# SamsungLabs/nb-asr

Measured on NVIDIA B200. Metric: train_utterances_per_sec, higher is better.
Workload: dtype bf16

## Files before the change

include/nbasr.h:

```cpp
#ifndef NBASR_H
#define NBASR_H

#include <stdint.h>

#ifdef __cplusplus
extern "C" {
#endif

#define NBASR_F32 0
#define NBASR_BF16 1
#define NBASR_F16 2
#define NBASR_PAD_L 8
#define NBASR_PAD_R 4
#define NBASR_MAX_ADD 3

typedef struct nbasr_epilogue {
  const float* bias;
  int32_t relu20;
  float drop_p;
  uint64_t drop_seed;
  const uint64_t* drop_step;
  int32_t n_add;
  const void* add[NBASR_MAX_ADD];
  int32_t add_dtype;
// ... 47 lines not shown
  const void* x;
  int32_t B, T, Tp, C, cpg, ktaps, off0, dstep;
  const void* w;
  int32_t w_packed;
  nbasr_epilogue epi;
} nbasr_gconv;

int nbasr_gconv_fwd(const nbasr_gconv* p, void* stream);
int nbasr_gconv_chain(const nbasr_gconv* nodes, int n, int fused, void* work, int64_t work_bytes, void* stream);
int64_t nbasr_gconv_chain_work_bytes(int B, int T, int C, int cpg, int n);
int nbasr_pack_gconv_dgrad(const float* w, float* wt, int C, int cpg, int ktaps, void* stream);
int nbasr_pack_gconv_mma(const float* w, void* out, int out_dtype, int C, int cpg, int ktaps, int transposed, void* stream);
int64_t nbasr_gconv_mma_pack_elems(int C, int cpg, int ktaps);
int nbasr_gconv_wgrad(int dtype, const void* dz, const void* x, int B, int T, int Tp, int C, int cpg,
                      int ktaps, int off0, int dstep, float* dw, float* dbias, void* stream);

int nbasr_eltwise(int src_dtype, const void* src, int64_t ld_src, int B, int T, int Tp, int C,
                  const nbasr_epilogue* epi, void* stream);

int nbasr_colsum(int dtype, const void* x, int B, int T, int Tp, int C, float* out, void* stream);

int nbasr_layernorm_fwd(int dtype, const void* x, void* y, int B, int T, int Tp, int C,
                        const float* gamma, const float* beta, float eps, float* mean, float* rstd,
                        float out_scale, void* y2, void* stream);
int nbasr_layernorm_bwd(int dtype, const void* dy, const void* x, int x_dtype, float x_scale, const float* mean,
                        const float* rstd, const float* gamma, int B, int T, int Tp, int C, void* dx, void* dx2,
                        const uint32_t* mask2, float scale2, int64_t mask_rows, int mask2_w, float* dgamma,
                        float* dbeta, void* stream);

int nbasr_transpose_in(const float* audio, void* out, int dtype, int B, int F, int T, int Tp, float scale, void* stream);
// ... 86 lines not shown
```

nb_asr_b200/_lib.py:

```python
import ctypes as C
import os

from . import _build

F32, BF16, F16 = 0, 1, 2
PAD_L, PAD_R = 8, 4
MAX_ADD = 3

_vp, _i32, _i64, _f32, _u64 = C.c_void_p, C.c_int32, C.c_int64, C.c_float, C.c_uint64


class Epilogue(C.Structure):
    _fields_ = [('bias', _vp), ('relu20', _i32), ('drop_p', _f32), ('drop_seed', _u64), ('drop_step', _vp),
                ('n_add', _i32), ('add', _vp * MAX_ADD), ('add_dtype', _i32), ('out', _vp), ('out_dtype', _i32),
                ('ld_out', _i64), ('mask_out', _vp), ('out2', _vp), ('out2_dtype', _i32), ('mask2', _vp),
                ('scale2', _f32), ('mask_rows', _i64), ('mask_w', _i32), ('mask2_w', _i32), ('accumulate', _i32),
                ('acc_scale', _f32), ('bias_scale', _f32), ('relu_hi', _f32)]


class Gemm(C.Structure):
    _fields_ = [('dtype', _i32), ('a', _vp), ('a_bs', _i64), ('a_rs', _i64), ('nb', _i32), ('nr', _i32),
                ('K', _i32), ('N', _i32), ('w', _vp), ('ldw', _i64), ('o_r0', _i64), ('o_bs', _i64),
                ('o_rs', _i64), ('epi', Epilogue)]

# ... 15 lines not shown
class GateLayer(C.Structure):
    _fields_ = [('mask', _vp), ('mask_rows', _i64), ('w', _i32), ('C', _i32), ('Tp', _i32), ('T', _i32), ('s', _i32),
                ('reserved', _i32)]


_SIGS = {
    'nbasr_gemm_tn': [C.POINTER(Gemm), _vp],
    'nbasr_gemm_wgrad': [C.POINTER(Wgrad), _vp],
    'nbasr_gconv_fwd': [C.POINTER(GConv), _vp],
    'nbasr_gconv_chain': [C.POINTER(GConv), C.c_int, C.c_int, _vp, _i64, _vp],
    'nbasr_gconv_chain_work_bytes': [C.c_int] * 5,
    'nbasr_pack_gconv_dgrad': [_vp, _vp, C.c_int, C.c_int, C.c_int, _vp],
    'nbasr_pack_gconv_mma': [_vp, _vp, C.c_int, C.c_int, C.c_int, C.c_int, C.c_int, _vp],
    'nbasr_gconv_mma_pack_elems': [C.c_int, C.c_int, C.c_int],
    'nbasr_gconv_wgrad': [C.c_int, _vp, _vp] + [C.c_int] * 8 + [_vp, _vp, _vp],
    'nbasr_eltwise': [C.c_int, _vp, _i64, C.c_int, C.c_int, C.c_int, C.c_int, C.POINTER(Epilogue), _vp],
    'nbasr_colsum': [C.c_int, _vp, C.c_int, C.c_int, C.c_int, C.c_int, _vp, _vp],
    'nbasr_layernorm_fwd': [C.c_int, _vp, _vp, C.c_int, C.c_int, C.c_int, C.c_int, _vp, _vp, _f32, _vp, _vp, _f32, _vp, _vp],
    'nbasr_layernorm_bwd': [C.c_int, _vp, _vp, C.c_int, _f32, _vp, _vp, _vp, C.c_int, C.c_int, C.c_int, C.c_int, _vp, _vp, _vp,
                            _f32, _i64, C.c_int, _vp, _vp, _vp],
    'nbasr_transpose_in': [_vp, _vp, C.c_int, C.c_int, C.c_int, C.c_int, C.c_int, _f32, _vp],
    'nbasr_transpose_out': [_vp, _vp, C.c_int, C.c_int, C.c_int, C.c_int, _vp],
    'nbasr_param_stats': [_vp, _vp, _vp, _vp, C.c_int, _i64, _vp, _vp, _vp],
    'nbasr_row_gram': [_vp, C.c_int, _i64, _i64, _vp, _vp, _vp, _vp],
    'nbasr_gate_gram': [_vp, C.c_int, _vp, C.c_int, _vp, _vp, _vp],
    'nbasr_gate_gram_work_elems': [C.c_int],
    'nbasr_pack_weight': [_vp, _vp, C.c_int, C.c_int, C.c_int, C.c_int, C.c_int, C.c_int, _i64, _i64, _i64, _vp],
    'nbasr_convert': [_vp, _vp, C.c_int, _i64, _vp],
    'nbasr_lstm_fwd': [_vp, _vp, C.c_int, C.c_int, C.c_int, _vp, C.c_int, _i64, _i64, _i64, _vp, _vp, _vp, _vp, _vp],
    'nbasr_lstm_bwd': [_vp, _i64, _i64, _i64, _vp, _vp, _vp, C.c_int, C.c_int, C.c_int, _vp, _vp, _vp, _vp, _vp],
# ... 60 lines not shown
```

nb_asr_b200/csrc/gconv.cu:

```cuda
#include <algorithm>

#include "common.cuh"
#include "kernels.h"

namespace {

constexpr int G_TT = 64;
constexpr int G_FB = 16;
constexpr int G_MAXHALO = 12;
constexpr int G_NT = 256;

__host__ __device__ inline int slab_channels(int cpg) {
  return cpg == 10 ? 160 : 96;
}
__host__ __device__ inline int wpitch(int cpg, int ktaps) {
  int p = cpg * ktaps;
  return (p & 1) ? p : p + 1;
}

template <typename T>
__global__ void __launch_bounds__(G_NT) gconv_fwd_kernel(nbasr_gconv p) {
  extern __shared__ float smem[];
  const int CS = slab_channels(p.cpg);
  const int halo = (p.ktaps - 1) * p.dstep;
// ... 69 lines not shown
  for (int item = tid; item < G_TT * nch; item += G_NT) {
    int r = item / nch, ch = item % nch;
    int t = t0 + r;
    if (t >= p.T) continue;
    float v[32];
#pragma unroll
    for (int i = 0; i < 32; ++i) v[i] = (ch * 32 + i < cs) ? os[r * (CS + 1) + ch * 32 + i] : 0.f;
    int64_t rho = (int64_t)b * p.Tp + NBASR_PAD_L + t;
    epilogue_chunk(p.epi, rho, c_lo + ch * 32, p.C, v);
  }
}

constexpr int W_PAIRS = 7;
constexpr int W_FB = 8;

template <typename T>
__global__ void __launch_bounds__(G_NT) gconv_wgrad_kernel(const T* __restrict__ dz, const T* __restrict__ x, int B,
                                                           int Tt, int Tp, int C, int cpg, int ktaps, int off0,
                                                           int dstep, float* __restrict__ dw) {
  extern __shared__ float smem[];
  const int CS = slab_channels(cpg);
  const int halo = (ktaps - 1) * dstep;
  float* xs = smem;
  float* ds = xs + (G_TT + G_MAXHALO) * CS;
  const int tid = threadIdx.x;
  const int c_lo = blockIdx.x * CS;
  const int cs = min(CS, C - c_lo);
  const int b = blockIdx.y;
  const int npairs = cs * cpg;
  float acc[W_PAIRS][7];
#pragma unroll
  for (int q = 0; q < W_PAIRS; ++q)
#pragma unroll
    for (int j = 0; j < 7; ++j) acc[q][j] = 0.f;
  const int vec = cs >> 3;
  for (int t0 = 0; t0 < Tt; t0 += G_TT) {
    __syncthreads();
    for (int idx = tid; idx < (G_TT + halo) * vec; idx += G_NT) {
      int r = idx / vec, g8 = idx % vec;
      int t = t0 + off0 + r;
      float v[8];
      if (t >= 0 && t < Tt) load8(x + ((int64_t)b * Tp + NBASR_PAD_L + t) * C + c_lo + g8 * 8, v);
      else {
#pragma unroll
        for (int i = 0; i < 8; ++i) v[i] = 0.f;
      }
#pragma unroll
      for (int i = 0; i < 8; ++i) xs[r * CS + g8 * 8 + i] = v[i];
    }
    for (int idx = tid; idx < G_TT * vec; idx += G_NT) {
      int r = idx / vec, g8 = idx % vec;
      int t = t0 + r;
      float v[8];
      if (t < Tt) load8(dz + ((int64_t)b * Tp + NBASR_PAD_L + t) * C + c_lo + g8 * 8, v);
      else {
#pragma unroll
        for (int i = 0; i < 8; ++i) v[i] = 0.f;
      }
#pragma unroll
      for (int i = 0; i < 8; ++i) ds[r * CS + g8 * 8 + i] = v[i];
    }
    __syncthreads();
#pragma unroll
// ... 90 lines not shown
  if (packed) return sm100_gconv_chain(nodes, n, fused, work, work_bytes, as_stream(stream));
  for (int i = 0; i < n; ++i)
    if (nbasr_gconv_fwd(nodes + i, stream)) return 1;
  return 0;
}

int64_t nbasr_gconv_chain_work_bytes(int B, int T, int C, int cpg, int n) { return sm100_gconv_chain_work_bytes(B, T, C, cpg, n); }

int nbasr_pack_gconv_dgrad(const float* w, float* wt, int C, int cpg, int ktaps, void* stream) {
  int total = C * cpg * ktaps;
  pack_gconv_dgrad_kernel<<<(total + 255) / 256, 256, 0, as_stream(stream)>>>(w, wt, C, cpg, ktaps);
  NBASR_CHECK_LAUNCH();
  return 0;
}

int nbasr_gconv_wgrad(int dtype, const void* dz, const void* x, int B, int T, int Tp, int C, int cpg, int ktaps,
                      int off0, int dstep, float* dw, float* dbias, void* stream) {
  NBASR_REQUIRE(cpg == 6 || cpg == 8 || cpg == 10 || cpg == 12, "cpg");
  NBASR_REQUIRE(ktaps <= 7 && (dstep == 1 || dstep == 2), "taps");
  if (B <= 0 || T <= 0) return 0;
  if (dtype == NBASR_BF16 && !nbasr_env_flag(NBASR_ENV_FORCE_SIMT))
    return sm100_gconv_wgrad(dz, x, B, T, Tp, C, cpg, ktaps, off0, dstep, dw, dbias, as_stream(stream));
  if (dbias && nbasr_colsum(dtype, dz, B, T, Tp, C, dbias, stream)) return 1;
  int CS = slab_channels(cpg);
  dim3 grid((C + CS - 1) / CS, B);
  size_t sm = wgrad_smem(cpg);
  if (dtype == NBASR_BF16) {
    static DevOnce attr;
    if (!attr) { cudaFuncSetAttribute(gconv_wgrad_kernel<bf16>, cudaFuncAttributeMaxDynamicSharedMemorySize, 200 * 1024); attr = true; }
    gconv_wgrad_kernel<bf16><<<grid, G_NT, sm, as_stream(stream)>>>((const bf16*)dz, (const bf16*)x, B, T, Tp, C, cpg, ktaps, off0, dstep, dw);
  } else {
    static DevOnce attr;
    if (!attr) { cudaFuncSetAttribute(gconv_wgrad_kernel<float>, cudaFuncAttributeMaxDynamicSharedMemorySize, 200 * 1024); attr = true; }
    gconv_wgrad_kernel<float><<<grid, G_NT, sm, as_stream(stream)>>>((const float*)dz, (const float*)x, B, T, Tp, C, cpg, ktaps, off0, dstep, dw);
  }
  NBASR_CHECK_LAUNCH();
  return 0;
}

}
```

nb_asr_b200/csrc/gconv_sm100.cu:

```cuda
#include <cuda.h>

#include "common.cuh"
#include "kernels.h"
#include "sm100_ptx.cuh"
#include "gconv_sm100.cuh"

using namespace sm100;

namespace {

struct GcFwdArgs {
  int B, T, C, OUT, ktaps, dstep, off0;
  int nslabs, ntiles, tiles_per_utt, nlanes, nstage, no_prefetch, w_stable, f16;
  nbasr_epilogue epi;
  int64_t Tp;
};


__global__ void __launch_bounds__(FWD_THREADS, 2)
gconv_mma_fwd_kernel(const __grid_constant__ CUtensorMap tmX, const __grid_constant__ CUtensorMap tmW,
                     const __grid_constant__ CUtensorMap tmO, const __grid_constant__ CUtensorMap tmO2, const GcFwdArgs p) {
  extern __shared__ uint8_t smem_raw[];
  const uint32_t base = (smem_u32(smem_raw) + 1023u) & ~1023u;
  uint8_t* al = smem_raw + (base - smem_u32(smem_raw));
// ... 212 lines not shown
  __syncthreads();
  if (warp == W_MMA) {
    tcgen05_fence_after();
    tmem_dealloc(tm, 256);
  }
}

constexpr int DZROWS = 136;
constexpr int DZ_BYTES = DZROWS * 128;
constexpr int WG_STAGE = DZ_BYTES + A_BYTES;
constexpr int WG_SMEM = NSTAGE * WG_STAGE + 1024 + 256;

struct GcWgArgs {
  int B, T, C, cpg, OUT, ktaps, dstep, off0;
  int nslabs, nchunks, nunits, nlanes, dbg;
  float* dw;
  float* dbias;
};

__global__ void __launch_bounds__(GC_THREADS, 2)
gconv_mma_wgrad_kernel(const __grid_constant__ CUtensorMap tmDZ, const __grid_constant__ CUtensorMap tmX, const GcWgArgs p) {
  extern __shared__ uint8_t smem_raw[];
  const uint32_t base = (smem_u32(smem_raw) + 1023u) & ~1023u;
  uint8_t* al = smem_raw + (base - smem_u32(smem_raw));
  const uint32_t bar0 = base + NSTAGE * WG_STAGE;
  auto full_bar = [&](int s) { return bar0 + 8u * s; };
  auto empty_bar = [&](int s) { return bar0 + 8u * (NSTAGE + s); };
  const uint32_t tfull = bar0 + 8u * (2 * NSTAGE);
  auto ready_bar = [&](int s) { return bar0 + 8u * (2 * NSTAGE + 1 + s); };
  uint32_t* tptr = reinterpret_cast<uint32_t*>(al + NSTAGE * WG_STAGE + 8 * (3 * NSTAGE + 2));
  const int warp = uniform_warp_idx(), lane = threadIdx.x & 31;
  const int slab = blockIdx.x % p.nslabs;
  const int lane_id = blockIdx.x / p.nslabs;
  const int c0 = slab * p.OUT;
  const int cbox = c0 & ~7, coff = c0 - cbox;
  const int npairs = (p.ktaps + 1) / 2;

  if (warp == 4 && lane == 0) {
    prefetch_tmap(&tmDZ);
    prefetch_tmap(&tmX);
    for (int s = 0; s < NSTAGE; ++s) { mbar_init(full_bar(s), 1); mbar_init(empty_bar(s), 1); mbar_init(ready_bar(s), 1); }
    mbar_init(tfull, 1);
    fence_barrier_init();
  }
  if (warp == 5) tmem_alloc(smem_u32(tptr), 256);
  pdl_launch_dependents();
  tcgen05_fence_before();
  __syncthreads();
  tcgen05_fence_after();
  const uint32_t tm = *tptr;
  pdl_wait();
  const bool has_work = lane_id < p.nunits;

  if (warp == 4) {
    if (lane == 0) {
      int stage = 0;
// ... 3 lines not shown
        mbar_wait(empty_bar(stage), phase ^ 1);
        mbar_expect_tx(full_bar(stage), DZ_BYTES + A_BYTES);
        const uint32_t sa = base + stage * WG_STAGE;
        tma_load_3d(sa, &tmDZ, full_bar(stage), cbox, NBASR_PAD_L + t0 - p.dstep, b);
        tma_load_3d(sa + DZ_BYTES, &tmX, full_bar(stage), cbox, NBASR_PAD_L + t0 + p.off0, b);
        if (++stage == NSTAGE) { stage = 0; phase ^= 1; }
      }
    }
  } else if (warp == 5) {
    if (has_work) {
      const uint32_t idesc = make_idesc(128, 64 * npairs, 1, 1);
      int stage = 0;
      uint32_t phase = 0;
      bool first = true;
      for (int u = lane_id; u < p.nunits; u += p.nlanes) {
        mbar_wait(p.dbias ? ready_bar(stage) : full_bar(stage), phase);
        const uint32_t sa = base + stage * WG_STAGE;
        tcgen05_fence_after();
        const uint64_t ad0 = make_smem_desc(sa, (uint32_t)p.dstep * 128u, 1024);
        const uint64_t bd0 = make_smem_desc(sa + DZ_BYTES, 2u * (uint32_t)p.dstep * 128u, 1024);
        if (elect_one()) {
#pragma unroll
          for (int k = 0; k < GT / 16; ++k)
            if (!(p.dbg & 2048) || k == 0) umma_bf16(tm, ad0 + (uint64_t)(k * 128), bd0 + (uint64_t)(k * 128), idesc, (!first || k > 0) ? 1u : 0u);
          umma_commit(empty_bar(stage));
        }
        __syncwarp();
        first = false;
        if (++stage == NSTAGE) { stage = 0; phase ^= 1; }
      }
      if (elect_one()) umma_commit(tfull);
      __syncwarp();
    }
  } else if (has_work) {
    if (warp == 0 && p.dbias) {
      int stage = 0;
      uint32_t phase = 0;
      for (int u = lane_id; u < p.nunits; u += p.nlanes) {
        mbar_wait(full_bar(stage), phase);
        uint8_t* xb = al + stage * WG_STAGE + DZ_BYTES;
        for (int r = lane; r < AROWS; r += 32)
          *reinterpret_cast<uint16_t*>(xb + r * 128 + ((7 ^ (r & 7)) << 4) + 14) = 0x3F80;
        asm volatile("fence.proxy.async.shared::cta;" ::: "memory");
        __syncwarp();
        if (lane == 0) mbar_arrive(ready_bar(stage));
        if (++stage == NSTAGE) { stage = 0; phase ^= 1; }
      }
    }
    const int q = warp & 3;
    const int m = q * 32 + lane;
    const int half = m >> 6, co_l = m & 63;
    const int co = cbox + co_l;
    const bool row_ok = co_l >= coff && co_l < coff + p.OUT && co < p.C;
    const int g_l = (co_l - coff) / p.cpg;
    mbar_wait(tfull, 0);
    tcgen05_fence_after();
    for (int pr = 0; pr < npairs; ++pr) {
      float v[64];
      const uint32_t ta = tm + ((uint32_t)(q * 32) << 16) + pr * 64;
      tmem_ld32(ta, v);
      tmem_ld32(ta + 32, v + 32);
      const int tap = half ? 2 * pr : 2 * pr + 1;
      if (pr == 0 && p.dbias && row_ok && half) atomicAdd(p.dbias + co, v[63]);
      if (row_ok && tap < p.ktaps && !(p.dbg & 1024)) {
        float* dst = p.dw + ((int64_t)co * p.cpg) * p.ktaps + tap;
#pragma unroll
        for (int i = 0; i < 64; ++i) {
          const int il = i - coff - g_l * p.cpg;
          if (il >= 0 && il < p.cpg) atomicAdd(dst + il * p.ktaps, v[i]);
        }
      }
    }
  }
  tcgen05_fence_before();
  __syncthreads();
  if (warp == 5) {
    tcgen05_fence_after();
    tmem_dealloc(tm, 256);
  }
}

template <typename T>
__global__ void pack_gconv_mma_kernel(const float* __restrict__ w, T* __restrict__ out, int C, int cpg, int ktaps, int OUT,
                                      int nslabs, int transposed) {
  int64_t idx = (int64_t)blockIdx.x * blockDim.x + threadIdx.x;
  int64_t total = (int64_t)nslabs * ktaps * NW * 64;
// ... 48 lines not shown
  if (sm100_get_map(o1, 3, dx, sx, bo, &tmO, 0)) return 1;
  if (sm100_get_map(o2, 3, dx, sx, bo, &tmO2, 0)) return 1;
  NBASR_REQUIRE(!g->epi.mask_out || g->epi.mask_w == a.OUT, "grouped-conv mask planes are slab wide");
  size_t smem = (size_t)a.ktaps * WTAP_BYTES + (size_t)a.nstage * A_BYTES + 2 * OSTAGE_BYTES + 1024 + 256 + 1024;
  static DevOnce attr;
  if (!attr) {
    cudaError_t e = cudaFuncSetAttribute(gconv_mma_fwd_kernel, cudaFuncAttributeMaxDynamicSharedMemorySize, FWD_SMEM_BUDGET);
    if (e != cudaSuccess) return nbasr_fail("gconv_mma_fwd smem attr: %s", cudaGetErrorString(e));
    attr = true;
  }
  cudaError_t le = launch_pdl(gconv_mma_fwd_kernel, dim3(a.nslabs * a.nlanes), dim3(FWD_THREADS), smem, st, 1, tmX, tmW, tmO, tmO2, a);
  if (le != cudaSuccess) return nbasr_fail("gconv_mma_fwd launch: %s", cudaGetErrorString(le));
  return 0;
}

int sm100_gconv_wgrad(const void* dz, const void* x, int B, int T, int Tp, int C, int cpg, int ktaps, int off0, int dstep,
                      float* dw, float* dbias, cudaStream_t st) {
  GcWgArgs a{};
  a.B = B; a.T = T; a.C = C; a.cpg = cpg; a.OUT = wg_slab_out(cpg); a.ktaps = ktaps; a.dstep = dstep; a.off0 = off0;
  NBASR_REQUIRE(off0 >= -NBASR_PAD_L && (ktaps - 1) * dstep <= AROWS - GT && dstep <= DZROWS - GT, "tap reach");
  a.nslabs = (C + a.OUT - 1) / a.OUT;
  a.nchunks = (T + dstep + GT - 1) / GT;
  a.nunits = a.nchunks * B;
  int slots = GCONV_SLOTS * nbasr_sm_count();
  a.nlanes = std::max(1, std::min(a.nunits, slots / a.nslabs));
  a.dw = dw;
  a.dbias = dbias;
  a.dbg = nbasr_env_chain_dbg();
  CUtensorMap tmDZ, tmX;
  uint64_t dd[3] = {(uint64_t)C, (uint64_t)Tp, (uint64_t)B};
  int64_t sd[3] = {1, C, (int64_t)Tp * C};
  uint32_t bz[3] = {64, DZROWS, 1};
  uint32_t bx[3] = {64, AROWS, 1};
// ... 30 lines not shown
```

nb_asr_b200/csrc/kernels.h:

```cpp
#pragma once
#include <cuda_runtime.h>
#include <stdint.h>

#include "../../include/nbasr.h"

enum NbasrEnvFlag { NBASR_ENV_FORCE_SIMT = 0, NBASR_ENV_NO_PDL, NBASR_ENV_GCONV_NO_PREFETCH, NBASR_ENV_LSTM_SS, NBASR_ENV_DEBUG,
                    NBASR_ENV_GEMM_DIRECT_EPI, NBASR_ENV_WGRAD_V1, NBASR_ENV_COUNT };
bool nbasr_env_flag(int which);
int nbasr_env_gemm_bn();
int nbasr_env_gemm_l2pf();
int nbasr_env_chain_dbg();
double nbasr_env_wgrad_epi_us();

struct DevOnce {
  unsigned long long mask = 0;
  static int dev() { int d = 0; cudaGetDevice(&d); return d & 63; }
  bool operator!() const { return !((mask >> dev()) & 1ull); }
  DevOnce& operator=(bool v) { if (v) mask |= 1ull << dev(); return *this; }
};

#ifdef __CUDACC__
#include <utility>
template <typename... KArgs, typename... Args>
inline cudaError_t launch_pdl(void (*kern)(KArgs...), dim3 grid, dim3 block, size_t smem, cudaStream_t st, int cluster_x,
// ... 29 lines not shown
  int64_t o_r0, o_bs, o_rs;
  nbasr_epilogue epi;
};
int simt_gemm_launch(const SimtGemmArgs& a, cudaStream_t st);

int sm100_gemm_tn_pair(const nbasr_gemm* p, cudaStream_t st);
int sm100_gemm_wgrad_pair(const nbasr_wgrad* p, cudaStream_t st);

struct CUtensorMap_st;
int sm100_get_map(const void* base, int rank, const uint64_t* dims, const int64_t* strides_el, const uint32_t* box,
                  CUtensorMap_st* out, int swizzle128 = 1);

int sm100_gconv_fwd(const nbasr_gconv* p, cudaStream_t st);
int sm100_gconv_chain(const nbasr_gconv* nodes, int n, int fused, void* work, int64_t work_bytes, cudaStream_t st);
int64_t sm100_gconv_chain_work_bytes(int B, int T, int C, int cpg, int n);
int sm100_gconv_wgrad(const void* dz, const void* x, int B, int T, int Tp, int C, int cpg, int ktaps, int off0, int dstep,
                      float* dw, float* dbias, cudaStream_t st);

int sm100_lstm_fwd(const float* gx, const void* w_packed, int T, int B, int H, void* h_seq, int h_dtype, int64_t h_bs, int64_t h_rs,
                   float* gates, float* cstate, cudaStream_t st);
int sm100_lstm_bwd(const float* dh_seq, int64_t dh_bs, int64_t dh_rs, const void* w_packed, const float* gates, const float* cstate,
                   int T, int B, int H, float* dgx, void* dgx_bf16, cudaStream_t st);

int ln2_fwd(const void* x, void* y, int f16, int B, int T, int Tp, int C, const float* gamma, const float* beta, float eps, float* mean,
            float* rstd, float out_scale, void* y2, cudaStream_t st);
int ln2_bwd(const void* dy, const void* x, int x_f16, float x_scale, const float* mean, const float* rstd, const float* gamma, int B, int T,
            int Tp, int C, void* dx, void* dx2, const uint32_t* mask2, float scale2, int64_t mask_rows, int mask2_w, float* dgamma,
            float* dbeta, cudaStream_t st);
```

nb_asr_b200/engine.py:

```python
import collections
import ctypes as C
import functools
import math
import os

import torch

from . import _lib
from ._lib import BF16, F16, F32, PAD_L, PAD_R, Epilogue, GConv, Gemm, Wgrad
from .model import CELLS_PER_BLOCK, CONV_EDGES, FEATURES, FILTERS, HIDDEN, TR_STRIDES, PadConvRelu, pad_rule

HP = 512
ACT_SCALE = 32.0


def _ptr(t, off_elems=0):
    return t.data_ptr() + off_elems * t.element_size()


class _Geo:

    def __init__(self, B, T, C):
        self.B, self.T, self.C = B, T, C
        tp = T + PAD_L + PAD_R
        self.Tp = tp + (tp & 1)
        self.rows = B * self.Tp + 8
        self.mw = (C + 31) // 32


class _Plan:
    pass

# ... 365 lines not shown
        grad = grad or input_grad
        key = (B, T, bool(training), grad) + (('input_grad',) if input_grad else ())
        pl = self.plans.get(key)
        if pl is None:
            while len(self.plans) >= max(1, self.max_plans):
                _, old = self.plans.popitem(last=False)
                old.graphs.clear()
                old.ws.clear()
            pl = self.plans[key] = self._build_plan(B, T, bool(training), grad, input_grad)
        else:
            self.plans.move_to_end(key)
        return pl

    def _plan_bytes_estimate(self, B, T, grad):
        es = 2 if self.dt == BF16 else 4
        total, Tcur = B * (T + 16) * FEATURES * es * 2, T
        for i in range(4):
            Tcur = Tcur if TR_STRIDES[i] == 1 else (Tcur + 1) // 2
            rows = B * (Tcur + PAD_L + PAD_R + 1) + 8
            per = rows * FILTERS[i] * es
            nbuf = 2 + 4 * CELLS_PER_BLOCK[i]
            total += per * nbuf
            if grad:
                total += per * (nbuf * (1 if self.adt != self.dt else 0) + 7) + per * nbuf // (8 * es) + per // 4
        total += B * Tcur * (4 * HIDDEN * 4 * (3 if grad else 1) + HP * 2 + HIDDEN * 4 * 3 + 49 * 4 * 3)
        return int(total * 1.05) + (8 << 20)

    @_on_device
    def _build_plan(self, B, T, training, grad=True, input_grad=False):
        self.bind()
        m, lib, dev, dt, tdt = self.model, self.lib, self.device, self.dt, self.tdt
        es = 2 if dt == BF16 else 4
        pl = _Plan()
        pl.B, pl.T, pl.training, pl.grad, pl.input_grad = B, T, training, grad, input_grad
        pl.keep = []
        pl.graphs, pl.ws = {}, {}
        arena = pl.arena = _Arena(dev, self._plan_bytes_estimate(B, T, grad))
        fwd, bwd_rev = [], []
        drop_p = self.training_drop if training else 0.0
        dscale = 1.0 / (1.0 - drop_p) if drop_p > 0 else 1.0
        salt = [1]

        def next_salt():
            salt[0] += 1
            return salt[0] * 0x9E3779B1

        adt, tadt, S = self.adt, self.tadt, self.S
        bcopy = {}

        def zbuf(rows, cols, dtype=None):
            return arena.zeros((rows, cols), tdt if dtype is None else dtype)

        def zact(rows, cols, copy=False):
            t = arena.zeros((rows, cols), tadt)
            if copy and grad and adt != dt:
                bcopy[id(t)] = arena.zeros((rows, cols), tdt)
            return t

        def Bc(t):
            return bcopy.get(id(t), t)

        def cptr(t):
            c = bcopy.get(id(t))
            return c.data_ptr() if c is not None else 0

        def call(lst, fn, *args):
            pl.keep.append(args)
            lst.append((fn, args))

        def gemm(lst, a_ptr, a_bs, a_rs, nb, nr, K, N, w_ptr, ldw, o_r0, o_bs, o_rs, epi, dtype=None):
            g = Gemm()
            g.dtype = dt if dtype is None else dtype
            g.a, g.a_bs, g.a_rs, g.nb, g.nr, g.K, g.N = a_ptr, a_bs, a_rs, nb, nr, K, N
            g.w, g.ldw, g.o_r0, g.o_bs, g.o_rs, g.epi = w_ptr, ldw, o_r0, o_bs, o_rs, epi
            call(lst, lib.nbasr_gemm_tn, C.byref(g))
# ... 13 lines not shown
            tt = tt if s_ == 1 else (tt + 1) // 2
            t_blk.append(tt)
        wbytes = max(int(lib.nbasr_gconv_chain_work_bytes(B, t_blk[i_], FILTERS[i_], FILTERS[i_] // 100, 3)) for i_ in range(4))
        pl.chain_work = arena.zeros(((wbytes + 3) // 4,), torch.int32)

        def flush_chain(lst, chain):
            if not chain:
                return
            arr = (GConv * len(chain))(*chain)
            fused = 1 if self.fuse_chains == 1 or self.fuse_chains == (2 if lst is fwd else 3) else 0
            call(lst, lib.nbasr_gconv_chain, arr, len(chain), fused, pl.chain_work.data_ptr(), pl.chain_work.numel() * 4)
            del chain[:]

        pl.audio = arena.zeros((B, FEATURES, T), torch.float32)
        g_in = _Geo(B, T, FEATURES)
        x_in = zact(g_in.rows, FEATURES, copy=True)
        call(fwd, lib.nbasr_transpose_in, pl.audio.data_ptr(), x_in.data_ptr(), adt, B, FEATURES, T, g_in.Tp, S)
        if cptr(x_in):
            call(fwd, lib.nbasr_transpose_in, pl.audio.data_ptr(), cptr(x_in), dt, B, FEATURES, T, g_in.Tp, 1.0)

        prev, pg = x_in, g_in
        Tcur = T
        arch = m.arch_desc
        pl.block_geo = []
        pl.gates = [] if grad else None
        gpools = []
        block_records = []
        for i in range(4):
            s = TR_STRIDES[i]
            Ti = Tcur if s == 1 else (Tcur + 1) // 2
            geo = _Geo(B, Ti, FILTERS[i])
            pl.block_geo.append(geo)
            Cc, Tp, mw = geo.C, geo.Tp, geo.mw
            cname = self.block_conv[i]
            lpad, _ = pad_rule(8, 1, s)
            K = 8 * pg.C
            z = zact(geo.rows, Cc)
            zmask = _Mask(geo.rows, Cc, 32, arena) if grad else None
            pl.keep.append(zmask)
            if grad:
                pl.gates.append((zmask, geo, i))
            wf_ptr = self.wf[cname].data_ptr() if self.wf[cname] is not None else self.P(cname + '.weight')
            a_ptr = _ptr(prev, (PAD_L - lpad) * pg.C)
            a_ptr_b = _ptr(Bc(prev), (PAD_L - lpad) * pg.C)
            epi = self._epi(Cc, bias=self.P(cname + '.bias'), relu=1, out=z.data_ptr(), mask_out=zmask, mask_rows=geo.rows, fwd=True)
            gemm(fwd, a_ptr, pg.Tp * pg.C, s * pg.C, B, Ti, K, Cc, wf_ptr, K, PAD_L, Tp, 1, epi, dtype=adt)
            n_ops = [nd[0] != 'zero' for nd in arch]
            y = zact(geo.rows, Cc, copy=True)
            mean0 = zbuf(geo.rows, 1, torch.float32)
            rstd0 = zbuf(geo.rows, 1, torch.float32)
            lname = self.block_ln[i]
            call(fwd, lib.nbasr_layernorm_fwd, adt, z.data_ptr(), y.data_ptr(), B, Ti, Tp, Cc, self.P(lname + '.weight'),
                 self.P(lname + '.bias'), 1e-3 * S * S, mean0.data_ptr(), rstd0.data_ptr(), S, cptr(y) or None)
            rec = dict(i=i, geo=geo, prev=prev, pg=pg, z=z, zmask=zmask, y=y, mean=mean0, rstd=rstd0, cells=[],
                       a_ptr=a_ptr_b, K=K, s=s, lpad=lpad)
            cur = y
            for cellname in self.block_cells[i]:
                outs = [cur]
                crec = dict(name=cellname, outs=outs, masks=[], nodes=[])
                chain = []
                for n, node in enumerate(arch):
                    op, branches = node[0], node[1:]
                    src = outs[-1]
                    skips = [outs[k] for k, bit in enumerate(branches) if bit]
                    o = zact(geo.rows, Cc, copy=(n_ops[n + 1] if n + 1 < len(arch) else not m.use_norm))
                    pn = f'{cellname}.nodes.{n}.op'
                    nrec = dict(op=op, branches=list(branches), pn=pn, mask=None, salt=0)
                    adds = [t.data_ptr() for t in skips]
                    if op not in CONV_EDGES:
                        flush_chain(fwd, chain)
                    if op == 'zero':
                        epi = self._epi(Cc, adds=adds, out=o.data_ptr(), fwd=True, copy=cptr(o))
                        call(fwd, lib.nbasr_eltwise, adt, None, Cc, B, Ti, Tp, Cc, C.byref(epi))
                        pl.keep.append(epi)
                    else:
                        mwid = (40 if Cc // 100 == 10 else 48) if (op in CONV_EDGES and dt == BF16) else 32
                        mask = _Mask(geo.rows, Cc, mwid, arena) if grad else None
                        pl.keep.append(mask)
                        nrec['mask'] = mask
                        if grad:
# ... 11 lines not shown
                            gc.dtype, gc.x, gc.B, gc.T, gc.Tp, gc.C, gc.cpg = adt, src.data_ptr(), B, Ti, Tp, Cc, Cc // 100
                            gc.ktaps, gc.off0, gc.dstep = k, -lp, d
                            if dt == BF16:
                                gc.w, gc.w_packed = self.wf[pn].data_ptr(), 3
                            else:
                                gc.w, gc.w_packed = self.P(pn + '.conv.weight'), 0
                            gc.epi = self._epi(Cc, bias=self.P(pn + '.conv.bias'), relu=1, drop_p=drop_p, salt=sl, adds=adds,
                                               out=o.data_ptr(), mask_out=mask, mask_rows=geo.rows, fwd=True, copy=cptr(o))
                            chain.append(gc)
                            pl.keep.append(gc)
                            nrec.update(k=k, d=d, lp=lp)
                    crec['nodes'].append(nrec)
                    outs.append(o)
                flush_chain(fwd, chain)
                if m.use_norm:
                    co = zact(geo.rows, Cc, copy=True)
                    mean = zbuf(geo.rows, 1, torch.float32)
                    rstd = zbuf(geo.rows, 1, torch.float32)
                    call(fwd, lib.nbasr_layernorm_fwd, adt, outs[-1].data_ptr(), co.data_ptr(), B, Ti, Tp, Cc,
                         self.P(cellname + '.norm_layer.weight'), self.P(cellname + '.norm_layer.bias'), 1e-3 * S * S,
                         mean.data_ptr(), rstd.data_ptr(), S, cptr(co) or None)
                    crec.update(mean=mean, rstd=rstd, out=co)
                    cur = co
                else:
                    crec.update(out=outs[-1])
                    cur = outs[-1]
                rec['cells'].append(crec)
            block_records.append(rec)
            prev, pg, Tcur = cur, geo, Ti

        geo3 = pl.block_geo[-1]
        Tq, Tp3, C3 = geo3.T, geo3.Tp, geo3.C
        pl.Tq = Tq
        V = m.num_classes + 1
        pl.V = V
        pl.logits = arena.zeros((B, Tq, V), torch.float32)
        pl.logp = arena.zeros((B, Tq, V), torch.float32)
        hn = self.head_name
        head = dict()
        if m.use_rnn:
            ln = self.lstm_name
            if drop_p > 0:
                lin = zact(geo3.rows, C3, copy=True)
                dmask = _Mask(geo3.rows, C3, 32, arena)
                pl.keep.append(dmask)
                epi = self._epi(C3, drop_p=drop_p, salt=next_salt(), out=lin.data_ptr(), mask_out=dmask, mask_rows=geo3.rows,
                                fwd=True, copy=cptr(lin))
                call(fwd, lib.nbasr_eltwise, adt, prev.data_ptr(), C3, B, Tq, Tp3, C3, C.byref(epi))
                pl.keep.append(epi)
            else:
                lin, dmask = prev, None
            H4 = 4 * HIDDEN
            gx = zbuf(B * Tq, H4, torch.float32)
            wih = self.wf[ln].data_ptr() if self.wf[ln] is not None else self.P(ln + '.weight_ih_l0')
            epi = self._epi(H4, bias=self.lstm_bias.data_ptr(), out=gx.data_ptr(), out_dtype=F32, acc_scale=1.0 / S)
            gemm(fwd, _ptr(lin, PAD_L * C3), Tp3 * C3, C3, B, Tq, C3, H4, wih, C3, 0, Tq, 1, epi, dtype=adt)
            gh = _Geo(B, Tq, HP)
            hseq = zbuf(gh.rows, HP)
# ... 105 lines not shown
                         self.G(crec['name'] + '.norm_layer.weight'), self.G(crec['name'] + '.norm_layer.bias'))
                    pool.append(gout)
                else:
                    g[nn_] = gout
                    if last['op'] != 'zero':
                        dz_t = dz[nn_ - 1]
                        dzb[nn_ - 1] = dz_t
                        epi = self._epi(Cc, out2=dz_t.data_ptr(), mask2=last['mask'], scale2=dscale, mask_rows=geo.rows)
                        call(bwd, lib.nbasr_eltwise, dt, gout.data_ptr(), Cc, B, Ti, Tp, Cc, C.byref(epi))
                        pl.keep.append(epi)
                chain, chain_wg = [], []

                def flush_bwd():
                    flush_chain(bwd, chain)
                    for a_ in chain_wg:
                        call(bwd, lib.nbasr_gconv_wgrad, *a_)
                    del chain_wg[:]

                for j in range(nn_ - 1, -1, -1):
                    nrec = nodes[j]
                    op, pn = nrec['op'], nrec['pn']
                    src = outs[j]
                    adds = [g[k + 1].data_ptr() for k in range(j, nn_) if nodes[k]['branches'][j]]
                    g[j] = pool.pop()
                    o2, m2 = 0, None
                    if j >= 1 and nodes[j - 1]['op'] != 'zero':
                        dzb[j - 1] = dz[j - 1]
                        o2, m2 = dzb[j - 1].data_ptr(), nodes[j - 1]['mask']
                    epi = self._epi(Cc, adds=adds, out=g[j].data_ptr() if (need_g(j) or not o2) else 0, out2=o2, mask2=m2, scale2=dscale,
                                    mask_rows=geo.rows)
                    if op not in CONV_EDGES:
                        flush_bwd()
                    if op == 'zero':
                        call(bwd, lib.nbasr_eltwise, dt, None, Cc, B, Ti, Tp, Cc, C.byref(epi))
                        pl.keep.append(epi)
                    elif op == 'linear':
                        d = dzb[j]
                        fuse = dt == BF16
                        wgrad(bwd, _ptr(d, PAD_L * Cc), Tp * Cc, Cc, _ptr(Bc(src), PAD_L * Cc), Tp * Cc, Cc, B, Ti, Cc, Cc,
                              self.G(pn + '.linear.weight'), Cc, dbias=self.G(pn + '.linear.bias') if fuse else None)
                        if not fuse:
                            call(bwd, lib.nbasr_colsum, dt, d.data_ptr(), B, Ti, Tp, Cc, self.G(pn + '.linear.bias'))
                        gemm(bwd, _ptr(d, PAD_L * Cc), Tp * Cc, Cc, B, Ti, Cc, Cc, self.wt[pn].data_ptr(), Cc, PAD_L, Tp, 1, epi)
                    else:
                        d = dzb[j]
                        k, dd, lp = nrec['k'], nrec['d'], nrec['lp']
                        chain_wg.append((dt, d.data_ptr(), Bc(src).data_ptr(), B, Ti, Tp, Cc, Cc // 100, k, -lp, dd,
                                         self.G(pn + '.conv.weight'), self.G(pn + '.conv.bias')))
                        gc = GConv()
                        gc.dtype, gc.x, gc.B, gc.T, gc.Tp, gc.C, gc.cpg = dt, d.data_ptr(), B, Ti, Tp, Cc, Cc // 100
                        gc.ktaps, gc.off0, gc.dstep, gc.w = k, lp - (k - 1) * dd, dd, self.wt[pn].data_ptr()
                        gc.w_packed = 3 if dt == BF16 else 0
                        gc.epi = epi
                        chain.append(gc)
                        pl.keep.append(gc)
                flush_bwd()
                for k in range(1, nn_ + 1):
                    pool.append(g[k])
                gout = g[0]
            dzc = dz[0]
            if i == 0:
                dz_blk0 = dzc
# ... 161 lines not shown
```

nb_asr_b200/profiling.py:

```python
import collections
import ctypes as C

import torch

from . import _lib
from ._lib import BF16, GConv, Gemm, Wgrad


def _struct_of(arg, typ):
    obj = getattr(arg, '_obj', None)
    return obj if isinstance(obj, typ) else None


def op_work(fn_name, args, es):
    if fn_name == 'nbasr_gemm_tn':
        g = _struct_of(args[0], Gemm)
        rows = g.nb * g.nr
        flops = 2.0 * rows * g.K * g.N
        a_cols = min(g.K, g.a_rs) if g.a_rs > 0 else g.K
        n_o = g.epi.n_add + (1 if g.epi.out else 0) + (1 if (g.epi.out2 and g.epi.mask2) else 0)
        byts = rows * a_cols * es + g.N * g.K * es + rows * g.N * es * n_o
        return f'gemm_tn K={g.K} N={g.N}', flops, byts
    if fn_name == 'nbasr_gemm_wgrad':
        w = _struct_of(args[0], Wgrad)
# ... 3 lines not shown
        byts = rows * (w.M + x_cols) * es + 4.0 * w.M * w.N * 2
        return f'gemm_wgrad M={w.M} N={w.N}', flops, byts
    if fn_name == 'nbasr_gconv_fwd':
        g = _struct_of(args[0], GConv)
        el = g.B * g.T * g.C
        n_t = 1 + g.epi.n_add + (1 if g.epi.out else 0) + (1 if (g.epi.out2 and g.epi.mask2) else 0)
        n_m = (1 if g.epi.mask_out else 0) + (1 if g.epi.mask2 else 0)
        return f'gconv C={g.C} k={g.ktaps} d={g.dstep}', 2.0 * el * g.cpg * g.ktaps, el * es * n_t + el * n_m / 8.0
    if fn_name == 'nbasr_gconv_chain':
        fl = by = 0.0
        for i in range(args[1]):
            _, f1, b1 = op_work('nbasr_gconv_fwd', (C.byref(args[0][i]),), es)
            fl, by = fl + f1, by + b1
        g = args[0][0]
        return f'gconv C={g.C} chain of {args[1]}', fl, by
    if fn_name == 'nbasr_gconv_wgrad':
        dt, dz, x, B, T, Tp, Cc, cpg, k = args[:9]
        el = B * T * Cc
        return f'gconv_wgrad C={Cc} k={k}', 2.0 * el * cpg * k, el * es * 2
    if fn_name in ('nbasr_layernorm_fwd', 'nbasr_layernorm_bwd'):
        if fn_name.endswith('fwd'):
            B, T, Tp, Cc = args[3:7]
            return f'ln_fwd C={Cc}', 0.0, B * T * Cc * es * 2
        B, T, Tp, Cc = args[8:12]
        n_out = (1 if args[12] else 0) + (1 if args[13] else 0)
        return f'ln_bwd C={Cc}', 0.0, B * T * Cc * es * (2 + n_out)
    if fn_name == 'nbasr_eltwise':
        B, T, Tp, Cc = args[3:7]
        return f'eltwise C={Cc}', 0.0, B * T * Cc * es * 2
    if fn_name == 'nbasr_colsum':
        B, T, Tp, Cc = args[2:6]
        return f'colsum C={Cc}', 0.0, B * T * Cc * (2 if args[0] == BF16 else 4)
# ... 52 lines not shown
```

Before: 8407.

## Feed fp16 activations directly to gconv wgrad and drop bf16 twin copies

The grouped-conv weight-gradient kernel can now read the fp16 forward activation directly. The conversion to bf16 and the scale by 1/S happen in shared memory, spread across four warps, so a bf16 twin copy of each conv input no longer has to be stored. Twin buffers are now kept only for inputs of linear (dense) wgrads. The dw epilogue also stages results in shared memory and flushes them with coalesced float4 atomics in place of per-element scattered atomics. The cost is extra in-kernel conversion work and a block-wide barrier, and scaling fp16 values could lose some precision.

```diff
diff --git a/include/nbasr.h b/include/nbasr.h
--- a/include/nbasr.h
+++ b/include/nbasr.h
@@ -85,6 +85,8 @@
 int64_t nbasr_gconv_mma_pack_elems(int C, int cpg, int ktaps);
 int nbasr_gconv_wgrad(int dtype, const void* dz, const void* x, int B, int T, int Tp, int C, int cpg,
                       int ktaps, int off0, int dstep, float* dw, float* dbias, void* stream);
+int nbasr_gconv_wgrad_x(int dz_dtype, const void* dz, const void* x, int x_dtype, float x_scale, int B, int T, int Tp, int C,
+                        int cpg, int ktaps, int off0, int dstep, float* dw, float* dbias, void* stream);
 
 int nbasr_eltwise(int src_dtype, const void* src, int64_t ld_src, int B, int T, int Tp, int C,
                   const nbasr_epilogue* epi, void* stream);
diff --git a/nb_asr_b200/_lib.py b/nb_asr_b200/_lib.py
--- a/nb_asr_b200/_lib.py
+++ b/nb_asr_b200/_lib.py
@@ -53,6 +53,7 @@
     'nbasr_pack_gconv_mma': [_vp, _vp, C.c_int, C.c_int, C.c_int, C.c_int, C.c_int, _vp],
     'nbasr_gconv_mma_pack_elems': [C.c_int, C.c_int, C.c_int],
     'nbasr_gconv_wgrad': [C.c_int, _vp, _vp] + [C.c_int] * 8 + [_vp, _vp, _vp],
+    'nbasr_gconv_wgrad_x': [C.c_int, _vp, _vp, C.c_int, _f32] + [C.c_int] * 8 + [_vp, _vp, _vp],
     'nbasr_eltwise': [C.c_int, _vp, _i64, C.c_int, C.c_int, C.c_int, C.c_int, C.POINTER(Epilogue), _vp],
     'nbasr_colsum': [C.c_int, _vp, C.c_int, C.c_int, C.c_int, C.c_int, _vp, _vp],
     'nbasr_layernorm_fwd': [C.c_int, _vp, _vp, C.c_int, C.c_int, C.c_int, C.c_int, _vp, _vp, _f32, _vp, _vp, _f32, _vp, _vp],
diff --git a/nb_asr_b200/csrc/gconv.cu b/nb_asr_b200/csrc/gconv.cu
--- a/nb_asr_b200/csrc/gconv.cu
+++ b/nb_asr_b200/csrc/gconv.cu
@@ -107,9 +107,9 @@
 constexpr int W_PAIRS = 7;
 constexpr int W_FB = 8;
 
-template <typename T>
-__global__ void __launch_bounds__(G_NT) gconv_wgrad_kernel(const T* __restrict__ dz, const T* __restrict__ x, int B,
-                                                           int Tt, int Tp, int C, int cpg, int ktaps, int off0,
+template <typename TD, typename TX>
+__global__ void __launch_bounds__(G_NT) gconv_wgrad_kernel(const TD* __restrict__ dz, const TX* __restrict__ x, float x_scale,
+                                                           int B, int Tt, int Tp, int C, int cpg, int ktaps, int off0,
                                                            int dstep, float* __restrict__ dw) {
   extern __shared__ float smem[];
   const int CS = slab_channels(cpg);
@@ -139,7 +139,7 @@
         for (int i = 0; i < 8; ++i) v[i] = 0.f;
       }
 #pragma unroll
-      for (int i = 0; i < 8; ++i) xs[r * CS + g8 * 8 + i] = v[i];
+      for (int i = 0; i < 8; ++i) xs[r * CS + g8 * 8 + i] = v[i] * x_scale;
     }
     for (int idx = tid; idx < G_TT * vec; idx += G_NT) {
       int r = idx / vec, g8 = idx % vec;
@@ -260,28 +260,34 @@
   return 0;
 }
 
-int nbasr_gconv_wgrad(int dtype, const void* dz, const void* x, int B, int T, int Tp, int C, int cpg, int ktaps,
-                      int off0, int dstep, float* dw, float* dbias, void* stream) {
+int nbasr_gconv_wgrad_x(int dz_dtype, const void* dz, const void* x, int x_dtype, float x_scale, int B, int T, int Tp, int C,
+                        int cpg, int ktaps, int off0, int dstep, float* dw, float* dbias, void* stream) {
   NBASR_REQUIRE(cpg == 6 || cpg == 8 || cpg == 10 || cpg == 12, "cpg");
   NBASR_REQUIRE(ktaps <= 7 && (dstep == 1 || dstep == 2), "taps");
+  NBASR_REQUIRE(dz_dtype == NBASR_BF16 ? (x_dtype == NBASR_BF16 || x_dtype == NBASR_F16) : (dz_dtype == NBASR_F32 && x_dtype == NBASR_F32),
+                "dtypes: bf16 dz with bf16 / fp16 x, or fp32 dz and x");
   if (B <= 0 || T <= 0) return 0;
-  if (dtype == NBASR_BF16 && !nbasr_env_flag(NBASR_ENV_FORCE_SIMT))
-    return sm100_gconv_wgrad(dz, x, B, T, Tp, C, cpg, ktaps, off0, dstep, dw, dbias, as_stream(stream));
-  if (dbias && nbasr_colsum(dtype, dz, B, T, Tp, C, dbias, stream)) return 1;
+  if (dz_dtype == NBASR_BF16 && !nbasr_env_flag(NBASR_ENV_FORCE_SIMT))
+    return sm100_gconv_wgrad(dz, x, x_dtype == NBASR_F16, x_scale, B, T, Tp, C, cpg, ktaps, off0, dstep, dw, dbias, as_stream(stream));
+  if (dbias && nbasr_colsum(dz_dtype, dz, B, T, Tp, C, dbias, stream)) return 1;
   int CS = slab_channels(cpg);
   dim3 grid((C + CS - 1) / CS, B);
   size_t sm = wgrad_smem(cpg);
-  if (dtype == NBASR_BF16) {
+  auto launch = [&](auto kern, auto dzp, auto xp) {
     static DevOnce attr;
-    if (!attr) { cudaFuncSetAttribute(gconv_wgrad_kernel<bf16>, cudaFuncAttributeMaxDynamicSharedMemorySize, 200 * 1024); attr = true; }
-    gconv_wgrad_kernel<bf16><<<grid, G_NT, sm, as_stream(stream)>>>((const bf16*)dz, (const bf16*)x, B, T, Tp, C, cpg, ktaps, off0, dstep, dw);
-  } else {
-    static DevOnce attr;
-    if (!attr) { cudaFuncSetAttribute(gconv_wgrad_kernel<float>, cudaFuncAttributeMaxDynamicSharedMemorySize, 200 * 1024); attr = true; }
-    gconv_wgrad_kernel<float><<<grid, G_NT, sm, as_stream(stream)>>>((const float*)dz, (const float*)x, B, T, Tp, C, cpg, ktaps, off0, dstep, dw);
-  }
+    if (!attr) { cudaFuncSetAttribute(kern, cudaFuncAttributeMaxDynamicSharedMemorySize, 200 * 1024); attr = true; }
+    kern<<<grid, G_NT, sm, as_stream(stream)>>>(dzp, xp, x_scale, B, T, Tp, C, cpg, ktaps, off0, dstep, dw);
+  };
+  if (dz_dtype == NBASR_F32) launch(gconv_wgrad_kernel<float, float>, (const float*)dz, (const float*)x);
+  else if (x_dtype == NBASR_F16) launch(gconv_wgrad_kernel<bf16, f16>, (const bf16*)dz, (const f16*)x);
+  else launch(gconv_wgrad_kernel<bf16, bf16>, (const bf16*)dz, (const bf16*)x);
   NBASR_CHECK_LAUNCH();
   return 0;
 }
 
-}
+int nbasr_gconv_wgrad(int dtype, const void* dz, const void* x, int B, int T, int Tp, int C, int cpg, int ktaps,
+                      int off0, int dstep, float* dw, float* dbias, void* stream) {
+  return nbasr_gconv_wgrad_x(dtype, dz, x, dtype, 1.f, B, T, Tp, C, cpg, ktaps, off0, dstep, dw, dbias, stream);
+}
+
+}
diff --git a/nb_asr_b200/csrc/gconv_sm100.cu b/nb_asr_b200/csrc/gconv_sm100.cu
--- a/nb_asr_b200/csrc/gconv_sm100.cu
+++ b/nb_asr_b200/csrc/gconv_sm100.cu
@@ -250,6 +250,8 @@
 struct GcWgArgs {
   int B, T, C, cpg, OUT, ktaps, dstep, off0;
   int nslabs, nchunks, nunits, nlanes, dbg;
+  int x_f16;
+  float x_scale;
   float* dw;
   float* dbias;
 };
@@ -275,7 +277,7 @@
   if (warp == 4 && lane == 0) {
     prefetch_tmap(&tmDZ);
     prefetch_tmap(&tmX);
-    for (int s = 0; s < NSTAGE; ++s) { mbar_init(full_bar(s), 1); mbar_init(empty_bar(s), 1); mbar_init(ready_bar(s), 1); }
+    for (int s = 0; s < NSTAGE; ++s) { mbar_init(full_bar(s), 1); mbar_init(empty_bar(s), 1); mbar_init(ready_bar(s), 4); }
     mbar_init(tfull, 1);
     fence_barrier_init();
   }
@@ -309,7 +311,7 @@
       uint32_t phase = 0;
       bool first = true;
       for (int u = lane_id; u < p.nunits; u += p.nlanes) {
-        mbar_wait(p.dbias ? ready_bar(stage) : full_bar(stage), phase);
+        mbar_wait((p.x_f16 || p.dbias) ? ready_bar(stage) : full_bar(stage), phase);
         const uint32_t sa = base + stage * WG_STAGE;
         tcgen05_fence_after();
         const uint64_t ad0 = make_smem_desc(sa, (uint32_t)p.dstep * 128u, 1024);
@@ -328,14 +330,33 @@
       __syncwarp();
     }
   } else if (has_work) {
-    if (warp == 0 && p.dbias) {
+    if (p.x_f16 || p.dbias) {
+      constexpr int QROWS = AROWS / 4;
+      const int r0 = warp * QROWS;
       int stage = 0;
       uint32_t phase = 0;
       for (int u = lane_id; u < p.nunits; u += p.nlanes) {
         mbar_wait(full_bar(stage), phase);
         uint8_t* xb = al + stage * WG_STAGE + DZ_BYTES;
-        for (int r = lane; r < AROWS; r += 32)
-          *reinterpret_cast<uint16_t*>(xb + r * 128 + ((7 ^ (r & 7)) << 4) + 14) = 0x3F80;
+        if (p.x_f16) {
+#pragma unroll 3
+          for (int i = lane; i < QROWS * 8; i += 32) {
+            const int r = r0 + (i >> 3), ch = i & 7;
+            uint4* cp = reinterpret_cast<uint4*>(xb + r * 128 + ch * 16);
+            uint4 w = *cp;
+            uint32_t* h = &w.x;
+#pragma unroll
+            for (int e = 0; e < 4; ++e) {
+              const float2 f = f16x2_to_f2(h[e]);
+              h[e] = f2_to_bf16x2(f.x * p.x_scale, f.y * p.x_scale);
+            }
+            if (p.dbias && ch == (7 ^ (r & 7))) w.w = (w.w & 0xffffu) | (0x3F80u << 16);
+            *cp = w;
+          }
+        } else {
+          for (int r = r0 + lane; r < r0 + QROWS; r += 32)
+            *reinterpret_cast<uint16_t*>(xb + r * 128 + ((7 ^ (r & 7)) << 4) + 14) = 0x3F80;
+        }
         asm volatile("fence.proxy.async.shared::cta;" ::: "memory");
         __syncwarp();
         if (lane == 0) mbar_arrive(ready_bar(stage));
@@ -348,6 +369,11 @@
     const int co = cbox + co_l;
     const bool row_ok = co_l >= coff && co_l < coff + p.OUT && co < p.C;
     const int g_l = (co_l - coff) / p.cpg;
+    const int nco = min(p.OUT, p.C - c0);
+    const int nrun = nco * p.cpg * p.ktaps;
+    float* g = p.dw + (int64_t)c0 * p.cpg * p.ktaps;
+    const int head = min(nrun, (int)(((16u - (uint32_t)(reinterpret_cast<uintptr_t>(g) & 15u)) & 15u) >> 2));
+    float* run = reinterpret_cast<float*>(al) + ((4 - head) & 3);
     mbar_wait(tfull, 0);
     tcgen05_fence_after();
     for (int pr = 0; pr < npairs; ++pr) {
@@ -357,14 +383,23 @@
       tmem_ld32(ta + 32, v + 32);
       const int tap = half ? 2 * pr : 2 * pr + 1;
       if (pr == 0 && p.dbias && row_ok && half) atomicAdd(p.dbias + co, v[63]);
-      if (row_ok && tap < p.ktaps && !(p.dbg & 1024)) {
-        float* dst = p.dw + ((int64_t)co * p.cpg) * p.ktaps + tap;
+      if (row_ok && tap < p.ktaps) {
+        float* dst = run + (co_l - coff) * p.cpg * p.ktaps + tap;
 #pragma unroll
         for (int i = 0; i < 64; ++i) {
           const int il = i - coff - g_l * p.cpg;
-          if (il >= 0 && il < p.cpg) atomicAdd(dst + il * p.ktaps, v[i]);
-        }
-      }
+          if (il >= 0 && il < p.cpg) dst[il * p.ktaps] = v[i];
+        }
+      }
+    }
+    named_bar_sync(1, 128);
+    if (!(p.dbg & 1024)) {
+      const int tid = threadIdx.x;
+      const int nvec = (nrun - head) >> 2, tail = head + 4 * nvec;
+      if (tid < head) atomicAdd(g + tid, run[tid]);
+      for (int j = tid; j < nvec; j += 128)
+        atomicAdd(reinterpret_cast<float4*>(g + head) + j, reinterpret_cast<const float4*>(run + head)[j]);
+      if (tail + tid < nrun) atomicAdd(g + tail + tid, run[tail + tid]);
     }
   }
   tcgen05_fence_before();
@@ -443,9 +478,11 @@
   return 0;
 }
 
-int sm100_gconv_wgrad(const void* dz, const void* x, int B, int T, int Tp, int C, int cpg, int ktaps, int off0, int dstep,
-                      float* dw, float* dbias, cudaStream_t st) {
+int sm100_gconv_wgrad(const void* dz, const void* x, int x_f16, float x_scale, int B, int T, int Tp, int C, int cpg, int ktaps,
+                      int off0, int dstep, float* dw, float* dbias, cudaStream_t st) {
   GcWgArgs a{};
+  a.x_f16 = x_f16;
+  a.x_scale = x_scale;
   a.B = B; a.T = T; a.C = C; a.cpg = cpg; a.OUT = wg_slab_out(cpg); a.ktaps = ktaps; a.dstep = dstep; a.off0 = off0;
   NBASR_REQUIRE(off0 >= -NBASR_PAD_L && (ktaps - 1) * dstep <= AROWS - GT && dstep <= DZROWS - GT, "tap reach");
   a.nslabs = (C + a.OUT - 1) / a.OUT;
diff --git a/nb_asr_b200/csrc/kernels.h b/nb_asr_b200/csrc/kernels.h
--- a/nb_asr_b200/csrc/kernels.h
+++ b/nb_asr_b200/csrc/kernels.h
@@ -67,8 +67,8 @@
 int sm100_gconv_fwd(const nbasr_gconv* p, cudaStream_t st);
 int sm100_gconv_chain(const nbasr_gconv* nodes, int n, int fused, void* work, int64_t work_bytes, cudaStream_t st);
 int64_t sm100_gconv_chain_work_bytes(int B, int T, int C, int cpg, int n);
-int sm100_gconv_wgrad(const void* dz, const void* x, int B, int T, int Tp, int C, int cpg, int ktaps, int off0, int dstep,
-                      float* dw, float* dbias, cudaStream_t st);
+int sm100_gconv_wgrad(const void* dz, const void* x, int x_f16, float x_scale, int B, int T, int Tp, int C, int cpg, int ktaps,
+                      int off0, int dstep, float* dw, float* dbias, cudaStream_t st);
 
 int sm100_lstm_fwd(const float* gx, const void* w_packed, int T, int B, int H, void* h_seq, int h_dtype, int64_t h_bs, int64_t h_rs,
                    float* gates, float* cstate, cudaStream_t st);
diff --git a/nb_asr_b200/engine.py b/nb_asr_b200/engine.py
--- a/nb_asr_b200/engine.py
+++ b/nb_asr_b200/engine.py
@@ -16,6 +16,22 @@
 
 def _ptr(t, off_elems=0):
     return t.data_ptr() + off_elems * t.element_size()
+
+
+def dense_wgrad_inputs(arch, use_norm, use_rnn, input_dropout=False):
+    ops = [nd[0] for nd in arch]
+    names = {'input'}
+    for i, ncells in enumerate(CELLS_PER_BLOCK):
+        cin = f'b{i}.ln'
+        for c in range(ncells):
+            outs = [cin] + [f'b{i}.c{c}.n{n}' for n in range(len(ops))]
+            names.update(outs[n] for n, op in enumerate(ops) if op == 'linear')
+            cin = f'b{i}.c{c}.ln' if use_norm else outs[-1]
+        if i < len(CELLS_PER_BLOCK) - 1:
+            names.add(cin)
+        elif use_rnn:
+            names.add('lstm_in' if input_dropout else cin)
+    return names
 
 
 class _Geo:
@@ -411,6 +427,7 @@
 
     def _plan_bytes_estimate(self, B, T, grad):
         es = 2 if self.dt == BF16 else 4
+        twins = dense_wgrad_inputs(self.model.arch_desc, self.model.use_norm, self.model.use_rnn) if self.adt != self.dt else ()
         total, Tcur = B * (T + 16) * FEATURES * es * 2, T
         for i in range(4):
             Tcur = Tcur if TR_STRIDES[i] == 1 else (Tcur + 1) // 2
@@ -419,7 +436,8 @@
             nbuf = 2 + 4 * CELLS_PER_BLOCK[i]
             total += per * nbuf
             if grad:
-                total += per * (nbuf * (1 if self.adt != self.dt else 0) + 7) + per * nbuf // (8 * es) + per // 4
+                ntw = sum(1 for n in twins if n.startswith(f'b{i}.'))
+                total += per * (ntw + 7) + per * nbuf // (8 * es) + per // 4
         total += B * Tcur * (4 * HIDDEN * 4 * (3 if grad else 1) + HP * 2 + HIDDEN * 4 * 3 + 49 * 4 * 3)
         return int(total * 1.05) + (8 << 20)
 
@@ -443,19 +461,22 @@
             return salt[0] * 0x9E3779B1
 
         adt, tadt, S = self.adt, self.tadt, self.S
+        twin_plan = grad and adt != dt
+        twin_names = dense_wgrad_inputs(m.arch_desc, m.use_norm, m.use_rnn, input_dropout=drop_p > 0) if twin_plan else ()
         bcopy = {}
+        pl.twins = {}
 
         def zbuf(rows, cols, dtype=None):
             return arena.zeros((rows, cols), tdt if dtype is None else dtype)
 
-        def zact(rows, cols, copy=False):
+        def zact(rows, cols, name=None):
             t = arena.zeros((rows, cols), tadt)
-            if copy and grad and adt != dt:
-                bcopy[id(t)] = arena.zeros((rows, cols), tdt)
+            if name in twin_names:
+                bcopy[id(t)] = pl.twins[name] = arena.zeros((rows, cols), tdt)
             return t
 
         def Bc(t):
-            return bcopy.get(id(t), t)
+            return bcopy[id(t)] if twin_plan else t
 
         def cptr(t):
             c = bcopy.get(id(t))
@@ -499,7 +520,7 @@
 
         pl.audio = arena.zeros((B, FEATURES, T), torch.float32)
         g_in = _Geo(B, T, FEATURES)
-        x_in = zact(g_in.rows, FEATURES, copy=True)
+        x_in = zact(g_in.rows, FEATURES, 'input')
         call(fwd, lib.nbasr_transpose_in, pl.audio.data_ptr(), x_in.data_ptr(), adt, B, FEATURES, T, g_in.Tp, S)
         if cptr(x_in):
             call(fwd, lib.nbasr_transpose_in, pl.audio.data_ptr(), cptr(x_in), dt, B, FEATURES, T, g_in.Tp, 1.0)
@@ -530,8 +551,7 @@
             a_ptr_b = _ptr(Bc(prev), (PAD_L - lpad) * pg.C)
             epi = self._epi(Cc, bias=self.P(cname + '.bias'), relu=1, out=z.data_ptr(), mask_out=zmask, mask_rows=geo.rows, fwd=True)
             gemm(fwd, a_ptr, pg.Tp * pg.C, s * pg.C, B, Ti, K, Cc, wf_ptr, K, PAD_L, Tp, 1, epi, dtype=adt)
-            n_ops = [nd[0] != 'zero' for nd in arch]
-            y = zact(geo.rows, Cc, copy=True)
+            y = zact(geo.rows, Cc, f'b{i}.ln')
             mean0 = zbuf(geo.rows, 1, torch.float32)
             rstd0 = zbuf(geo.rows, 1, torch.float32)
             lname = self.block_ln[i]
@@ -540,7 +560,7 @@
             rec = dict(i=i, geo=geo, prev=prev, pg=pg, z=z, zmask=zmask, y=y, mean=mean0, rstd=rstd0, cells=[],
                        a_ptr=a_ptr_b, K=K, s=s, lpad=lpad)
             cur = y
-            for cellname in self.block_cells[i]:
+            for ci, cellname in enumerate(self.block_cells[i]):
                 outs = [cur]
                 crec = dict(name=cellname, outs=outs, masks=[], nodes=[])
                 chain = []
@@ -548,7 +568,7 @@
                     op, branches = node[0], node[1:]
                     src = outs[-1]
                     skips = [outs[k] for k, bit in enumerate(branches) if bit]
-                    o = zact(geo.rows, Cc, copy=(n_ops[n + 1] if n + 1 < len(arch) else not m.use_norm))
+                    o = zact(geo.rows, Cc, f'b{i}.c{ci}.n{n}')
                     pn = f'{cellname}.nodes.{n}.op'
                     nrec = dict(op=op, branches=list(branches), pn=pn, mask=None, salt=0)
                     adds = [t.data_ptr() for t in skips]
@@ -590,7 +610,7 @@
                     outs.append(o)
                 flush_chain(fwd, chain)
                 if m.use_norm:
-                    co = zact(geo.rows, Cc, copy=True)
+                    co = zact(geo.rows, Cc, f'b{i}.c{ci}.ln')
                     mean = zbuf(geo.rows, 1, torch.float32)
                     rstd = zbuf(geo.rows, 1, torch.float32)
                     call(fwd, lib.nbasr_layernorm_fwd, adt, outs[-1].data_ptr(), co.data_ptr(), B, Ti, Tp, Cc,
@@ -617,7 +637,7 @@
         if m.use_rnn:
             ln = self.lstm_name
             if drop_p > 0:
-                lin = zact(geo3.rows, C3, copy=True)
+                lin = zact(geo3.rows, C3, 'lstm_in')
                 dmask = _Mask(geo3.rows, C3, 32, arena)
                 pl.keep.append(dmask)
                 epi = self._epi(C3, drop_p=drop_p, salt=next_salt(), out=lin.data_ptr(), mask_out=dmask, mask_rows=geo3.rows,
@@ -753,7 +773,7 @@
                 def flush_bwd():
                     flush_chain(bwd, chain)
                     for a_ in chain_wg:
-                        call(bwd, lib.nbasr_gconv_wgrad, *a_)
+                        call(bwd, lib.nbasr_gconv_wgrad_x, *a_)
                     del chain_wg[:]
 
                 for j in range(nn_ - 1, -1, -1):
@@ -784,7 +804,7 @@
                     else:
                         d = dzb[j]
                         k, dd, lp = nrec['k'], nrec['d'], nrec['lp']
-                        chain_wg.append((dt, d.data_ptr(), Bc(src).data_ptr(), B, Ti, Tp, Cc, Cc // 100, k, -lp, dd,
+                        chain_wg.append((dt, d.data_ptr(), src.data_ptr(), adt, 1.0 / S, B, Ti, Tp, Cc, Cc // 100, k, -lp, dd,
                                          self.G(pn + '.conv.weight'), self.G(pn + '.conv.bias')))
                         gc = GConv()
                         gc.dtype, gc.x, gc.B, gc.T, gc.Tp, gc.C, gc.cpg = dt, d.data_ptr(), B, Ti, Tp, Cc, Cc // 100
diff --git a/nb_asr_b200/profiling.py b/nb_asr_b200/profiling.py
--- a/nb_asr_b200/profiling.py
+++ b/nb_asr_b200/profiling.py
@@ -41,8 +41,8 @@
             fl, by = fl + f1, by + b1
         g = args[0][0]
         return f'gconv C={g.C} chain of {args[1]}', fl, by
-    if fn_name == 'nbasr_gconv_wgrad':
-        dt, dz, x, B, T, Tp, Cc, cpg, k = args[:9]
+    if fn_name in ('nbasr_gconv_wgrad', 'nbasr_gconv_wgrad_x'):
+        B, T, Tp, Cc, cpg, k = args[3:9] if fn_name == 'nbasr_gconv_wgrad' else args[5:11]
         el = B * T * Cc
         return f'gconv_wgrad C={Cc} k={k}', 2.0 * el * cpg * k, el * es * 2
     if fn_name in ('nbasr_layernorm_fwd', 'nbasr_layernorm_bwd'):
```

New measurement: 8821, median of 6. 1.05x the previous value.
